# visinf/fldr-vfi

Measured on AMD Instinct MI355X. Metric: 4K frame-pairs interpolated/sec, higher is better.
Workload: dtype f32 (3x3 convs: 3 x fp16-split MFMA with fp32 accumulation — error against fp64 within 1.5x (mean) / 2x (max) of the exact fp32-MFMA kernel's on every layer shape, tests/test_gpu_parity.py::test_split_fp16_conv_is_fp32_equivalent; rest fp32/fp64)

## Files before the change

### fldr-vfi_amd/csrc/splat_acc64_kernels.hip

```cpp
#include "splat_common.h"

#define SA_SBQ 64
#define SA_Q 512
#ifndef SA_WHOLE_PIXELS
#define SA_WHOLE_PIXELS 2304
#endif
#ifndef SA_IMG_TW
#define SA_IMG_TW 64
#define SA_IMG_TH 24
#define SA_IMG_K 3
#define SA_IMG_U 4
#endif
#ifndef SA_IMGQ_U
#define SA_IMGQ_U 1
#endif
#ifndef SA_FEAT_TW
#define SA_FEAT_TW 32
#define SA_FEAT_TH 8
#define SA_FEAT_K 1
#define SA_FEAT_U 1
#endif

typedef _Float16 sa_h8 __attribute__((ext_vector_type(8)));

struct SaProblem {
    const float* img;
    const float* flow;
    const float* metric;
    const float* blk;
    const float* sbt;
    float* out_f32;
    unsigned char* out_spk;
    int64_t img_bstride, img_cstride, flow_bstride;
};
struct SaArgs {
    SaProblem p[2];
    int N, C, H, W, groups, nsb_x, nsb;
    int whole;
    int gpw;
    int tiles_x, st_y, n_st, total, per_xcd;
};

template <int CB, int U, bool QUAD>
struct SaBuf {
    int x[U], y[U];
    bool ok[U];
    float fx[U], fy[U], mv[U], val[U][CB];
};
template <int CB, int U>
struct SaBuf<CB, U, true> {
    int x[U], y[U];
    bool ok[U];
    float4 fx[U], fy[U], mv[U], val[U][CB];
};
__device__ __forceinline__ void sa_pin4(float4& v) { fldr_pin(v.x); fldr_pin(v.y); fldr_pin(v.z); fldr_pin(v.w); }
__device__ __forceinline__ float sa_at(const float4& v, int j) { return j == 0 ? v.x : (j == 1 ? v.y : (j == 2 ? v.z : v.w)); }

template <int MODE, int CB, int TW, int TH, int K, int U, bool QUAD>
__global__ __launch_bounds__(256) void splat_acc64_kernel(SaArgs a) {
#pragma clang fp contract(off)
    constexpr int CA = MODE >= 1 ? CB + 1 : CB;
    constexpr int CELLS = TW * TH;
    extern __shared__ __attribute__((aligned(16))) unsigned char sa_smem[];
    double* acc = reinterpret_cast<double*>(sa_smem);
    int* blkq = reinterpret_cast<int*>(sa_smem + (size_t)CA * CELLS * 8);
    float* redf = reinterpret_cast<float*>(blkq + SA_Q);
    int* redi = reinterpret_cast<int*>(redf + 16);
    int* cnt = redi + 16;
    unsigned short* sbq = reinterpret_cast<unsigned short*>(cnt + 2);

    const int tid = threadIdx.x, lane = tid & 63;
    const int wv = __builtin_amdgcn_readfirstlane(tid >> 6);
    const int lin = (int)(blockIdx.x & 7) * a.per_xcd + (int)(blockIdx.x >> 3);
    if ((int)(blockIdx.x >> 3) >= a.per_xcd || lin >= a.total) return;
    const int zi = lin / a.n_st, st = lin - zi * a.n_st;
    const int sty = st / a.tiles_x, stx = st - sty * a.tiles_x;
    const int wg_groups = a.groups / a.gpw;
    const int per_prob = a.N * wg_groups;
    const int prob = zi / per_prob;
    const int rem = zi - prob * per_prob;
    const int n = rem / wg_groups, grp0 = (rem - n * wg_groups) * a.gpw;
    const SaProblem& P = a.p[prob];
    const int C = a.C, H = a.H, W = a.W, nsb_x = a.nsb_x, nsb = a.nsb;
    int cbase = grp0 * CB;
    const int tx0 = stx * TW, sy0 = sty * (K * TH);
    const int64_t HW = (int64_t)H * W;
    const float ftx0 = (float)tx0, ftx1 = (float)(tx0 + TW - 1), fsy0 = (float)sy0, fsy1 = (float)(min(sy0 + K * TH, H) - 1);
    const float INF = __builtin_inff();

    const float* sbn = P.sbt + (int64_t)n * nsb * 4;
    const float* bkn = P.blk + (int64_t)n * nsb * ST_SB_BLOCKS * 4;
    const bool small = nsb <= SA_SBQ;
    if (tid < 2) cnt[tid] = small && tid == 0 ? nsb : 0;
    if (small && tid < nsb) sbq[tid] = (unsigned short)tid;
    float4 b_first = make_float4(0.0f, 0.0f, 0.0f, 0.0f);
    if (!small && !a.whole) b_first = *reinterpret_cast<const float4*>(sbn + (tid < nsb ? tid : 0) * 4);
    for (int i = tid; i < CA * CELLS / 2; i += 256) reinterpret_cast<double2*>(acc)[i] = make_double2(0.0, 0.0);
    if ((CA * CELLS) & 1) { if (tid == 0) acc[CA * CELLS - 1] = 0.0; }
    __syncthreads();
    if (!small && !a.whole) {
        for (int s = tid; s < nsb; s += 256) {
            const float4 b = s == tid ? b_first : *reinterpret_cast<const float4*>(sbn + s * 4);
            const int sx = (s % nsb_x) * (ST_SBX * ST_BW), sy = (s / nsb_x) * (ST_SBY * ST_BH);
            if (st_match(b, (float)sx, (float)(sx + ST_SBX * ST_BW - 1), (float)sy, (float)(sy + ST_SBY * ST_BH - 1), ftx0, ftx1, fsy0, fsy1)) {
                const int i = atomicAdd(&cnt[0], 1);
                if (i < SA_SBQ) sbq[i] = (unsigned short)s;
            }
        }
        __syncthreads();
    }
    const int n_sb = cnt[0];
    const bool sb_over = a.whole || n_sb > SA_SBQ;
    float rxmin = INF, rxmax = -INF, rymin = INF, rymax = -INF;
    int cx0 = 0x7fffffff, cx1 = -1, cy0 = 0x7fffffff, cy1 = -1;
    if (!sb_over) {
        for (int i = wv; i < n_sb; i += 4) {
            const int s = sbq[i];
            const float4 b = *reinterpret_cast<const float4*>(bkn + ((int64_t)s * ST_SB_BLOCKS + lane) * 4);
            const int bx = (s % nsb_x) * ST_SBX + (lane % ST_SBX), by = (s / nsb_x) * ST_SBY + (lane / ST_SBX);
            const int sx = bx * ST_BW, sy = by * ST_BH;
            if (st_match(b, (float)sx, (float)(sx + ST_BW - 1), (float)sy, (float)(sy + ST_BH - 1), ftx0, ftx1, fsy0, fsy1)) {
                rxmin = fminf(rxmin, b.x); rxmax = fmaxf(rxmax, b.y); rymin = fminf(rymin, b.z); rymax = fmaxf(rymax, b.w);
                cx0 = min(cx0, sx); cx1 = max(cx1, sx + ST_BW - 1); cy0 = min(cy0, sy); cy1 = max(cy1, sy + ST_BH - 1);
                const int k = atomicAdd(&cnt[1], 1);
                if (k < SA_Q) blkq[k] = (by << 16) | bx;
            }
        }
#pragma unroll
        for (int o = 32; o > 0; o >>= 1) {
            rxmin = fminf(rxmin, __shfl_xor(rxmin, o)); rxmax = fmaxf(rxmax, __shfl_xor(rxmax, o));
            rymin = fminf(rymin, __shfl_xor(rymin, o)); rymax = fmaxf(rymax, __shfl_xor(rymax, o));
            cx0 = min(cx0, __shfl_xor(cx0, o)); cx1 = max(cx1, __shfl_xor(cx1, o));
            cy0 = min(cy0, __shfl_xor(cy0, o)); cy1 = max(cy1, __shfl_xor(cy1, o));
        }
        if (lane == 0) {
            redf[wv * 4 + 0] = rxmin; redf[wv * 4 + 1] = rxmax; redf[wv * 4 + 2] = rymin; redf[wv * 4 + 3] = rymax;
            redi[wv * 4 + 0] = cx0; redi[wv * 4 + 1] = cx1; redi[wv * 4 + 2] = cy0; redi[wv * 4 + 3] = cy1;
        }
    }
    __syncthreads();
    int n_match = 0;
    bool bounded = false;
    if (!sb_over) {
        n_match = cnt[1];
#pragma unroll
        for (int k = 0; k < 4; ++k) {
            rxmin = fminf(rxmin, redf[k * 4 + 0]); rxmax = fmaxf(rxmax, redf[k * 4 + 1]);
            rymin = fminf(rymin, redf[k * 4 + 2]); rymax = fmaxf(rymax, redf[k * 4 + 3]);
            cx0 = min(cx0, redi[k * 4 + 0]); cx1 = max(cx1, redi[k * 4 + 1]); cy0 = min(cy0, redi[k * 4 + 2]); cy1 = max(cy1, redi[k * 4 + 3]);
        }
        bounded = fabsf(rxmin) < 1.0e6f && fabsf(rxmax) < 1.0e6f && fabsf(rymin) < 1.0e6f && fabsf(rymax) < 1.0e6f;
    }

    const float* fl = P.flow + (int64_t)n * P.flow_bstride;
    const float* mt = P.metric ? P.metric + (int64_t)n * HW : nullptr;
    const float* inn = P.img + (int64_t)n * P.img_bstride;
    float* on = P.out_f32 ? P.out_f32 + (int64_t)n * C * HW : nullptr;
    const int G = (C + 7) >> 3;
    unsigned char* sp = P.out_spk ? P.out_spk + (int64_t)n * G * 2 * HW * 16 : nullptr;
    bool bad = false;

    int ty0 = 0;
    int X0 = 0, Y0 = 0, Rw = 1, Rh = 0, n_chunks = 0;
    bool rect = true;
    int rx = 0, ry = 0, dqx = 0, dqy = 0;
    auto plan_tile = [&](int k) __attribute__((always_inline)) {
        ty0 = sy0 + k * TH;
        const float fty0 = (float)ty0, fty1 = (float)(ty0 + TH - 1);
        int X1 = W - 1, Y1 = H - 1;
        X0 = 0; Y0 = 0; rect = true; n_chunks = 0;
        if (sb_over) {
            n_chunks = (int)((HW + 255) / 256);
        } else if (n_match > 0) {
            X0 = cx0; X1 = min(cx1, W - 1); Y0 = cy0; Y1 = min(cy1, H - 1);
            if (bounded) {
                X0 = max(X0, (int)floorf(ftx0 - 2.0f - rxmax)); X1 = min(X1, (int)ceilf(ftx1 + 1.0f - rxmin));
                Y0 = max(Y0, (int)floorf(fty0 - 2.0f - rymax)); Y1 = min(Y1, (int)ceilf(fty1 + 1.0f - rymin));
            }
            const int64_t area = (int64_t)max(X1 - X0 + 1, 0) * max(Y1 - Y0 + 1, 0);
            rect = n_match > SA_Q || area <= (int64_t)256 * n_match;
            n_chunks = rect ? (int)((area + 255) / 256) : n_match;
        }
        Rw = max(X1 - X0 + 1, 1); Rh = max(Y1 - Y0 + 1, 0);
        if constexpr (QUAD) {
            X0 &= ~3; X1 = min(X1 | 3, W - 1);
            Rw = max((X1 - X0 + 1) >> 2, 1);
            if (n_chunks > 0) n_chunks = rect ? (int)(((int64_t)Rw * Rh + 255) / 256) : (n_match + 3) >> 2;
        }
        rx = tid % Rw; ry = tid / Rw;
        dqx = 256 % Rw; dqy = 256 / Rw;
#if defined(SA_ABLATE) && SA_ABLATE == 1
        n_chunks = 0;
#endif
    };

    auto load_chunk = [&](SaBuf<CB, U, QUAD>& b, int u, int k) __attribute__((always_inline)) {
        int x, y;
        bool ok;
        if (rect) {
            x = X0 + (QUAD ? 4 * rx : rx); y = Y0 + ry;
            ok = k < n_chunks && ry < Rh;
            rx += dqx; ry += dqy;
            if (rx >= Rw) { rx -= Rw; ++ry; }
        } else if constexpr (QUAD) {
            const int bi = 4 * k + wv;
            const int e = blkq[bi < n_match ? bi : 0];
            x = (e & 0xFFFF) * ST_BW + (lane & 15) * 4; y = (e >> 16) * ST_BH + (lane >> 4);
            ok = bi < n_match && x < W && y < H;
        } else {
            const int e = blkq[k < n_chunks ? k : 0];
            x = (e & 0xFFFF) * ST_BW + lane; y = (e >> 16) * ST_BH + wv;
            ok = k < n_chunks && x < W && y < H;
        }
        b.x[u] = x; b.y[u] = y; b.ok[u] = ok;
        const int64_t pix = ok ? (int64_t)y * W + x : 0;
        if constexpr (QUAD) {
            b.fx[u] = *reinterpret_cast<const float4*>(fl + pix); b.fy[u] = *reinterpret_cast<const float4*>(fl + HW + pix);
            b.mv[u] = make_float4(0.0f, 0.0f, 0.0f, 0.0f);
            if ((MODE == 2 || MODE == 3) && mt != nullptr) b.mv[u] = *reinterpret_cast<const float4*>(mt + pix);
#pragma unroll
            for (int c = 0; c < CB; ++c) {
                const int cc = cbase + c < C ? cbase + c : C - 1;
                b.val[u][c] = *reinterpret_cast<const float4*>(inn + (int64_t)cc * P.img_cstride + pix);
            }
        } else {
            b.fx[u] = fl[pix]; b.fy[u] = fl[HW + pix];
            b.mv[u] = 0.0f;
            if ((MODE == 2 || MODE == 3) && mt != nullptr) b.mv[u] = mt[pix];
#pragma unroll
            for (int c = 0; c < CB; ++c) {
                const int cc = cbase + c < C ? cbase + c : C - 1;
                b.val[u][c] = inn[(int64_t)cc * P.img_cstride + pix];
            }
        }
    };
    auto load_iter = [&](SaBuf<CB, U, QUAD>& b, int k0) __attribute__((always_inline)) {
#pragma unroll
        for (int u = 0; u < U; ++u) load_chunk(b, u, k0 + u);
    };
    auto process = [&](SaBuf<CB, U, QUAD>& b) __attribute__((always_inline)) {
      if constexpr (QUAD) {
#pragma unroll
        for (int u = 0; u < U; ++u) {
            sa_pin4(b.fx[u]); sa_pin4(b.fy[u]); sa_pin4(b.mv[u]);
#pragma unroll
            for (int c = 0; c < CB; ++c) sa_pin4(b.val[u][c]);
        }
#if defined(SA_ABLATE) && SA_ABLATE == 3
        return;
#endif
#pragma unroll
        for (int u = 0; u < U; ++u) {
            if (!b.ok[u]) continue;
            int x0[4], y0[4], iw[4], ie[4];
            float wnw[4], wne[4], wsw[4], wse[4], wg[4];
            bool xa[4], xb[4], ya[4], yb[4];
            bool any = false;
#pragma unroll
            for (int j = 0; j < 4; ++j) {
                const StGeom g = st_geom(b.x[u] + j, b.y[u], sa_at(b.fx[u], j), sa_at(b.fy[u], j), W, H);
                x0[j] = g.x0; y0[j] = g.y0; wnw[j] = g.wnw; wne[j] = g.wne; wsw[j] = g.wsw; wse[j] = g.wse;
                const uint32_t ulx = (uint32_t)(g.x0 - tx0), uly = (uint32_t)(g.y0 - ty0), ux1 = ulx + 1u;
                xa[j] = ulx < (uint32_t)TW; xb[j] = ux1 < (uint32_t)TW; ya[j] = uly < (uint32_t)TH; yb[j] = uly + 1u < (uint32_t)TH;
                iw[j] = (int)(uly * (uint32_t)TW + (ulx & 3u) * (uint32_t)(TW / 4) + (ulx >> 2));
                ie[j] = (int)(uly * (uint32_t)TW + (ux1 & 3u) * (uint32_t)(TW / 4) + (ux1 >> 2));
                any = any || ((xa[j] || xb[j]) && (ya[j] || yb[j]));
                wg[j] = 1.0f;
                if (MODE == 2) wg[j] = sa_at(b.mv[u], j);
                if (MODE == 3 && mt != nullptr) wg[j] = expf(sa_at(b.mv[u], j));
            }
            if (!any) continue;
            float v[4][CA];
#pragma unroll
            for (int j = 0; j < 4; ++j)
#pragma unroll
                for (int c = 0; c < CA; ++c) {
                    float t = wg[j];
                    if (c < CB) {
                        t = sa_at(b.val[u][c < CB ? c : 0], j);
                        if (MODE == 3) t = (t + 1.0f) / 2.0f;
                        if (MODE >= 2) t = t * wg[j];
                        if (cbase + c >= C) t = 0.0f;
                    }
                    v[j][c] = t;
                }
            bool gn[4], gs[4];
#pragma unroll
            for (int j = 0; j < 4; ++j) {
                const bool coh = j < 3 && x0[j] + 1 == x0[j < 3 ? j + 1 : j] && y0[j] == y0[j < 3 ? j + 1 : j];
                gn[j] = coh && xb[j] && ya[j]; gs[j] = coh && xb[j] && yb[j];
            }
#pragma unroll
            for (int j = 0; j < 4; ++j) {
                const int jp = j > 0 ? j - 1 : 0;
                if (xa[j] && ya[j]) {
#pragma unroll
                    for (int c = 0; c < CA; ++c) {
                        double d = (double)(v[j][c] * wnw[j]);
                        if (j > 0) d += (double)(gn[jp] ? v[jp][c] * wne[jp] : 0.0f);
                        atomicAdd(acc + c * CELLS + iw[j], d);
                    }
                }
                if (xa[j] && yb[j]) {
#pragma unroll
                    for (int c = 0; c < CA; ++c) {
                        double d = (double)(v[j][c] * wsw[j]);
                        if (j > 0) d += (double)(gs[jp] ? v[jp][c] * wse[jp] : 0.0f);
                        atomicAdd(acc + c * CELLS + iw[j] + TW, d);
                    }
                }
                if (xb[j] && ya[j] && !gn[j]) {
#pragma unroll
                    for (int c = 0; c < CA; ++c) atomicAdd(acc + c * CELLS + ie[j], (double)(v[j][c] * wne[j]));
                }
                if (xb[j] && yb[j] && !gs[j]) {
#pragma unroll
                    for (int c = 0; c < CA; ++c) atomicAdd(acc + c * CELLS + ie[j] + TW, (double)(v[j][c] * wse[j]));
                }
            }
        }
      } else {
#pragma unroll
        for (int u = 0; u < U; ++u) {
            fldr_pin(b.fx[u]); fldr_pin(b.fy[u]); fldr_pin(b.mv[u]);
#pragma unroll
            for (int c = 0; c < CB; ++c) fldr_pin(b.val[u][c]);
        }
#if defined(SA_ABLATE) && SA_ABLATE == 3
        return;
#endif
#pragma unroll
        for (int u = 0; u < U; ++u) {
            if (!b.ok[u]) continue;
            const StGeom g = st_geom(b.x[u], b.y[u], b.fx[u], b.fy[u], W, H);
            const int lx = g.x0 - tx0, ly = g.y0 - ty0;
            if (lx < -1 || lx >= TW || ly < -1 || ly >= TH) continue;
            const bool cxa = lx >= 0 && g.x0 < W, cxb = lx + 1 < TW && g.x0 + 1 < W;
            const bool cya = ly >= 0 && g.y0 < H, cyb = ly + 1 < TH && g.y0 + 1 < H;
            const bool vnw = cxa && cya, vne = cxb && cya, vsw = cxa && cyb, vse = cxb && cyb;
            float wgt = 1.0f;
            if (MODE == 2) wgt = b.mv[u];
            if (MODE == 3 && mt != nullptr) wgt = expf(b.mv[u]);
            double* cell = acc + (ly * TW + lx);
#pragma unroll
            for (int c = 0; c < CA; ++c) {
                float v;
                if (c < CB) {
                    v = b.val[u][c];
                    if (MODE == 3) v = (v + 1.0f) / 2.0f;
                    if (MODE >= 2) v = v * wgt;
                    if (cbase + c >= C) v = 0.0f;
                } else {
                    v = wgt;
                }
                double* pc = cell + c * CELLS;
#if defined(SA_ABLATE) && SA_ABLATE == 2
                asm volatile("" :: "v"(pc), "v"(v * g.wnw), "v"(v * g.wne), "v"(v * g.wsw), "v"(v * g.wse), "v"((int)vnw + (int)vne + (int)vsw + (int)vse));
#else
                if (vnw) atomicAdd(pc, (double)(v * g.wnw));
                if (vne) atomicAdd(pc + 1, (double)(v * g.wne));
                if (vsw) atomicAdd(pc + TW, (double)(v * g.wsw));
                if (vse) atomicAdd(pc + TW + 1, (double)(v * g.wse));
#endif
            }
        }
      }
    };
    auto finish = [&](int fy0, int cbase) __attribute__((always_inline)) {
      if constexpr (QUAD) {
        static_assert(!QUAD || (CB % 8 != 0 && TW % 4 == 0), "the run walk serves the image configuration (fp32 output)");
        for (int i = tid; i < CELLS / 4; i += 256) {
            const int xq = i % (TW / 4), yy = i / (TW / 4);
            const int x = tx0 + 4 * xq, y = fy0 + yy;
            const int cell = yy * TW + xq;
            float norm[4] = {1.0f, 1.0f, 1.0f, 1.0f};
            if (MODE >= 1) {
#pragma unroll
                for (int j = 0; j < 4; ++j) {
                    norm[j] = (float)acc[CB * CELLS + cell + j * (TW / 4)]; acc[CB * CELLS + cell + j * (TW / 4)] = 0.0;
                    if (norm[j] == 0.0f) norm[j] = 1.0f;
                }
            }
            float o[CB][4];
            StRecip rn[4];
            bool fast = true;
            if (MODE >= 1) {
#pragma unroll
                for (int j = 0; j < 4; ++j) { rn[j] = st_recip(norm[j]); fast = fast && st_recip_safe(norm[j]); }
                fast = __builtin_amdgcn_ballot_w64(!fast) == 0ull;
            }
#pragma unroll
            for (int c = 0; c < CB; ++c)
#pragma unroll
                for (int j = 0; j < 4; ++j) {
                    float v = (float)acc[c * CELLS + cell + j * (TW / 4)];
                    acc[c * CELLS + cell + j * (TW / 4)] = 0.0;
                    if (MODE >= 1) v = fast ? st_div(v, rn[j]) : v / norm[j];
                    o[c][j] = (v - 0.5f) * 2.0f;
                }
            if (x >= W || y >= H || !on) continue;
            const int64_t pix = (int64_t)y * W + x;
#pragma unroll
            for (int c = 0; c < CB; ++c)
                if (cbase + c < C) *reinterpret_cast<float4*>(on + (int64_t)(cbase + c) * HW + pix) = make_float4(o[c][0], o[c][1], o[c][2], o[c][3]);
        }
      } else {
        for (int i = tid; i < CELLS; i += 256) {
            const int x = tx0 + i % TW, y = fy0 + i / TW;
            float norm = 1.0f;
            if (MODE >= 1) { norm = (float)acc[CB * CELLS + i]; acc[CB * CELLS + i] = 0.0; if (norm == 0.0f) norm = 1.0f; }
            float o[CB];
            const StRecip rn = st_recip(norm);
            const bool fast = MODE >= 1 && __builtin_amdgcn_ballot_w64(!st_recip_safe(norm)) == 0ull;
#pragma unroll
            for (int c = 0; c < CB; ++c) {
                float v = (float)acc[c * CELLS + i];
                acc[c * CELLS + i] = 0.0;
                if (MODE >= 1) v = fast ? st_div(v, rn) : v / norm;
                o[c] = cbase + c < C ? (v - 0.5f) * 2.0f : 0.0f;
            }
            if (x >= W || y >= H) continue;
            const int64_t pix = (int64_t)y * W + x;
            if (on) {
#pragma unroll
                for (int c = 0; c < CB; ++c)
                    if (cbase + c < C) on[(int64_t)(cbase + c) * HW + pix] = o[c];
            }
            if constexpr (CB % 8 == 0) {
                if (sp) {
#pragma unroll
                    for (int g8 = 0; g8 < CB / 8; ++g8) {
                        const int gi = (cbase >> 3) + g8;
                        if (gi >= G) break;
                        sa_h8 hi, lo;
                        {
                            float xs[8];
                            _Float16 hs[8], ls[8];
#pragma unroll
                            for (int k = 0; k < 8; ++k) xs[k] = o[g8 * 8 + k];
                            fldr_split_hl_group(xs, hs, ls, bad);
#pragma unroll
                            for (int k = 0; k < 8; ++k) { hi[k] = hs[k]; lo[k] = ls[k]; }
                        }
                        unsigned char* d = sp + ((int64_t)gi * 2 * HW + pix) * 16;
                        *reinterpret_cast<sa_h8*>(d) = hi;
                        *reinterpret_cast<sa_h8*>(d + HW * 16) = lo;
                    }
                }
            }
        }
      }
    };

    SaBuf<CB, U, QUAD> b0, b1;
    const int n_units = K * a.gpw;
    auto begin_unit = [&](int u) __attribute__((always_inline)) {
        const int k = u / a.gpw;
        cbase = (grp0 + (u - k * a.gpw)) * CB;
        plan_tile(k);
        if (n_chunks > 0) load_iter(b0, 0);
    };
    begin_unit(0);
#pragma unroll 1
    for (int u = 0; u < n_units; ++u) {
        const int cur_y0 = ty0, cur_cbase = cbase;
        if (cur_y0 >= H) break;
        for (int k0 = 0; k0 < n_chunks; k0 += 2 * U) {
            const bool more = k0 + U < n_chunks;
            if (more) load_iter(b1, k0 + U);
            process(b0);
            if (!more) break;
            if (k0 + 2 * U < n_chunks) load_iter(b0, k0 + 2 * U);
            process(b1);
        }
        const bool next = u + 1 < n_units && sy0 + ((u + 1) / a.gpw) * TH < H;
        if (next) begin_unit(u + 1);
        __syncthreads();
        finish(cur_y0, cur_cbase);
        if (!next) break;
        __syncthreads();
    }
    fldr_note_range(bad);
}

FLDR_TU_STATUS(acc64)

#ifndef SA_FOLD_MIN_TILES
#define SA_FOLD_MIN_TILES 512
#endif
#ifndef SA_QUAD_DEFAULT
#define SA_QUAD_DEFAULT 1
#endif
static int g_sa_quad = SA_QUAD_DEFAULT;
FLDR_HOOK int fldr_debug_splat_quad(int v) { if (v == 0 || v == 1) g_sa_quad = v; return g_sa_quad; }
static int g_sa_group_fold = 0;
FLDR_HOOK int fldr_debug_splat_group_fold(int v) { if (v == 0 || v == 1) g_sa_group_fold = v; return g_sa_group_fold; }

template <int MODE, int CB, int TW, int TH, int K, int U, bool QUAD = false>
static int sa_launch2(SaArgs& a, int nprob, hipStream_t s) {
    constexpr int CA = MODE >= 1 ? CB + 1 : CB;
    constexpr int LDS = CA * TW * TH * 8 + SA_Q * 4 + 16 * 4 + 16 * 4 + 2 * 4 + SA_SBQ * 2;
    static_assert(LDS <= 160 * 1024, "tile does not fit the LDS");
    static std::atomic<uint64_t> attr_done{0};
    if (int e = fldr_set_max_lds(reinterpret_cast<const void*>(&splat_acc64_kernel<MODE, CB, TW, TH, K, U, QUAD>), LDS, attr_done)) return e;
    a.tiles_x = fldr_cdiv(a.W, TW);
    a.st_y = fldr_cdiv(a.H, K * TH);
    a.n_st = a.tiles_x * a.st_y;
    const int64_t total = (int64_t)nprob * a.N * (a.groups / a.gpw) * a.n_st;
    if (total > (1ll << 30)) return FLDR_E_SHAPE;
    a.total = (int)total;
    a.per_xcd = (a.total + 7) / 8;
    hipLaunchKernelGGL((splat_acc64_kernel<MODE, CB, TW, TH, K, U, QUAD>), dim3(8 * a.per_xcd), dim3(256), LDS, s, a);
    return 0;
}

template <int MODE>
static int sa_launch(SaArgs& a, int nprob, hipStream_t s) {
    if (a.C <= 3) {
        a.groups = 1; a.gpw = 1;
        bool quad = g_sa_quad && a.W % 4 == 0;
        for (int k = 0; k < nprob && quad; ++k) {
            const SaProblem& p = a.p[k];
            quad = ((reinterpret_cast<uintptr_t>(p.img) | reinterpret_cast<uintptr_t>(p.flow) | reinterpret_cast<uintptr_t>(p.metric) |
                     reinterpret_cast<uintptr_t>(p.out_f32)) & 15) == 0 && ((p.img_bstride | p.img_cstride | p.flow_bstride) & 3) == 0 && p.out_spk == nullptr;
        }
        if (quad) return sa_launch2<MODE, 3, SA_IMG_TW, SA_IMG_TH, SA_IMG_K, SA_IMGQ_U, true>(a, nprob, s);
        return sa_launch2<MODE, 3, SA_IMG_TW, SA_IMG_TH, SA_IMG_K, SA_IMG_U>(a, nprob, s);
    }
    a.groups = fldr_cdiv(a.C, 16);
    const int64_t tiles = (int64_t)nprob * a.N * fldr_cdiv(a.W, SA_FEAT_TW) * fldr_cdiv(a.H, SA_FEAT_TH * SA_FEAT_K);
    a.gpw = (g_sa_group_fold && tiles >= SA_FOLD_MIN_TILES) ? a.groups : 1;
    return sa_launch2<MODE, 16, SA_FEAT_TW, SA_FEAT_TH, SA_FEAT_K, SA_FEAT_U>(a, nprob, s);
}

extern "C" int fldr_softsplat_acc64(const fldr_splat_acc_desc* d, fldr_stream_t stream) {
    FLDR_CHECK_ARG(d && d->nprob >= 1 && d->nprob <= 2 && d->N > 0 && d->C > 0 && d->H > 0 && d->W > 0 && d->mode >= 0 && d->mode <= 3);
    FLDR_CHECK_ARG(!(d->flags & ~7) && (!(d->flags & 2) || (d->nprob == 2 && !(d->flags & 1))));
    if (d->W > 65535 * ST_BW || d->H > 32767 * ST_BH || (int64_t)d->H * d->W * 4 >= (1ll << 32)) return FLDR_E_SHAPE;
    if ((int64_t)fldr_cdiv(d->W, ST_SBX * ST_BW) * fldr_cdiv(d->H, ST_SBY * ST_BH) > 65535) return FLDR_E_SHAPE;
    SaArgs a;
    a.N = d->N; a.C = d->C; a.H = d->H; a.W = d->W; a.groups = 1;
    a.whole = ((d->flags & 4) || (!(d->flags & 3) && (int64_t)d->H * d->W <= SA_WHOLE_PIXELS)) ? 1 : 0;
    a.nsb_x = fldr_cdiv(d->W, ST_SBX * ST_BW);
    a.nsb = a.nsb_x * fldr_cdiv(d->H, ST_SBY * ST_BH);
    hipStream_t s = fldr_s(stream);
    const int64_t HW = (int64_t)d->H * d->W;
    for (int k = 0; k < 2; ++k) {
        const int j = k < d->nprob ? k : 0;
        FLDR_CHECK_ARG(d->img[j] && d->flow[j] && (a.whole || d->ws[(d->flags & 2) ? 0 : j]) && (d->out_f32[j] || d->out_spk[j]));
        FLDR_CHECK_ARG(d->mode != 2 || d->metric[j] != nullptr);
        FLDR_CHECK_ARG(!d->out_spk[j] || d->C > 3);
        SaProblem& p = a.p[k];
        p.img = d->img[j]; p.flow = d->flow[j]; p.metric = d->metric[j];
        if (a.whole) {
            p.blk = p.sbt = nullptr;
// ... 24 lines not shown
```

### fldr-vfi_amd/csrc/splat_common.h

```cpp
#pragma once
#include "common.h"

#define ST_BW 64
#define ST_BH 4
#define ST_SBX 4
#define ST_SBY 16
#define ST_SB_BLOCKS (ST_SBX * ST_SBY)
#define ST_Q 1024
#define ST_SBQ 64
#define ST_U 4

struct StGeom {
    int   x0, y0;
    float wnw, wne, wsw, wse;
};

__device__ __forceinline__ StGeom st_geom(int x, int y, float fx, float fy, int W, int H) {
#pragma clang fp contract(off)
    StGeom g;
    float ox = (float)x + fx;
    float oy = (float)y + fy;
    float xf = floorf(ox), yf = floorf(oy);
    float x1 = xf + 1.0f, y1 = yf + 1.0f;
    g.wnw = (x1 - ox) * (y1 - oy);
    g.wne = (ox - xf) * (y1 - oy);
    g.wsw = (x1 - ox) * (oy - yf);
    g.wse = (ox - xf) * (oy - yf);
    xf = fminf(fmaxf(xf, -2.0f), (float)W + 1.0f);
    yf = fminf(fmaxf(yf, -2.0f), (float)H + 1.0f);
    g.x0 = (int)xf; g.y0 = (int)yf;
    return g;
}

struct StRecip { float n, r; };
__device__ __forceinline__ StRecip st_recip(float n) {
    StRecip q;
    q.n = n;
    const float r0 = __builtin_amdgcn_rcpf(n);
// ... 95 lines not shown
```

### fldr-vfi_amd/fldr_hip.py

```python
import ctypes
import os

import torch

_HERE = os.path.dirname(os.path.abspath(__file__))
LIB_PATH = os.environ.get("FLDR_LIB") or os.path.join(_HERE, "libfldr_hip.so")

MAX_SRC = 12
_c_float_p = ctypes.c_void_p


class ConvDesc(ctypes.Structure):
    _fields_ = [
        ("src", ctypes.c_void_p * MAX_SRC),
        ("src_bstride", ctypes.c_int64 * MAX_SRC),
        ("src_c", ctypes.c_int32 * MAX_SRC),
        ("src_up2", ctypes.c_int32 * MAX_SRC),
        ("n_src", ctypes.c_int32),
        ("wpack", ctypes.c_void_p),
        ("bias", ctypes.c_void_p),
        ("residual", ctypes.c_void_p),
        ("out", ctypes.c_void_p),
        ("N", ctypes.c_int32), ("cin", ctypes.c_int32), ("cout", ctypes.c_int32), ("cout_store", ctypes.c_int32),
        ("Hin", ctypes.c_int32), ("Win", ctypes.c_int32), ("Hout", ctypes.c_int32), ("Wout", ctypes.c_int32),
# ... 99 lines not shown
    "fldr_debug_s2_vec4": (ctypes.c_int, [ctypes.c_int]),
    "fldr_bwarp": (ctypes.c_int, [_c_float_p] * 3 + [ctypes.c_int] * 5 + [ctypes.c_void_p]),
    "fldr_bwarp_tscaled": (ctypes.c_int, [_c_float_p] * 4 + [ctypes.c_int] * 7 + [ctypes.c_void_p]),
    "fldr_resize_bilinear": (ctypes.c_int, [_c_float_p] * 2 + [ctypes.c_int] * 5 + [ctypes.c_float, ctypes.c_void_p]),
    "fldr_level0_prep": (ctypes.c_int, [ctypes.POINTER(PrepDesc), ctypes.c_void_p]),
    "fldr_zmetric": (ctypes.c_int, [_c_float_p] * 3 + [ctypes.c_float, _c_float_p] + [ctypes.c_int] * 4 + [ctypes.c_void_p]),
    "fldr_conv_prepack_size": (ctypes.c_int64, [ctypes.c_int] * 3),
    "fldr_conv_prepack": (ctypes.c_int, [_c_float_p] * 2 + [ctypes.c_int] * 3 + [ctypes.c_void_p]),
    "fldr_conv2d": (ctypes.c_int, [ctypes.POINTER(ConvDesc), ctypes.c_void_p]),
    "fldr_conv_split_prepack_size": (ctypes.c_int64, [ctypes.c_int] * 2),
    "fldr_conv_split_prepack": (ctypes.c_int, [_c_float_p] * 2 + [ctypes.c_int] * 2 + [ctypes.c_void_p]),
    "fldr_conv2d_split": (ctypes.c_int, [ctypes.POINTER(ConvDesc), ctypes.c_void_p]),
    "fldr_conv_s2_prepack_size": (ctypes.c_int64, [ctypes.c_int] * 2),
    "fldr_conv_s2_prepack": (ctypes.c_int, [_c_float_p] * 2 + [ctypes.c_int] * 2 + [ctypes.c_void_p]),
    "fldr_conv2d_s2_split": (ctypes.c_int, [ctypes.POINTER(ConvDesc), ctypes.c_void_p]),
    "fldr_conv2d_s2_spk": (ctypes.c_int, [ctypes.POINTER(ConvDesc), ctypes.c_void_p]),
    "fldr_conv2d_s2_spk_pair": (ctypes.c_int, [ctypes.POINTER(ConvDesc), ctypes.POINTER(ConvDesc), ctypes.c_void_p]),
    "fldr_debug_s2_persistent": (ctypes.c_int, [ctypes.c_int]),
    "fldr_debug_s2_dma": (ctypes.c_int, [ctypes.c_int]),
    "fldr_debug_s2_xshift": (ctypes.c_int, [ctypes.c_int]),
    "fldr_debug_dec3_xshift": (ctypes.c_int, [ctypes.c_int]),
    "fldr_debug_dec3_xcd": (ctypes.c_int, [ctypes.c_int]),
    "fldr_debug_splat_quad": (ctypes.c_int, [ctypes.c_int]),
    "fldr_spk_bytes": (ctypes.c_int64, [ctypes.c_int] * 3),
    "fldr_spk_pack": (ctypes.c_int, [_c_float_p, ctypes.c_int64, ctypes.c_void_p] + [ctypes.c_int] * 4 + [ctypes.c_void_p]),
    "fldr_spk_unpack": (ctypes.c_int, [ctypes.c_void_p, _c_float_p] + [ctypes.c_int] * 4 + [ctypes.c_void_p]),
    "fldr_conv_spk_prepack_size": (ctypes.c_int64, [ctypes.c_int] * 2),
    "fldr_conv_spk_prepack": (ctypes.c_int, [_c_float_p] * 2 + [ctypes.c_int] * 2 + [ctypes.c_void_p]),
    "fldr_conv2d_spk": (ctypes.c_int, [ctypes.POINTER(SpkConvDesc), ctypes.c_void_p]),
    "fldr_conv2d_spk_levels": (ctypes.c_int, [ctypes.POINTER(SpkConvDesc), ctypes.c_int, ctypes.c_void_p]),
    "fldr_debug_spk_wgs_per_xcd": (ctypes.c_int, [ctypes.c_int]),
    "fldr_range_status": (ctypes.c_int, [ctypes.c_int]),
    "fldr_ring_status": (ctypes.c_int, [ctypes.c_int]),
    "fldr_debug_spk_small_units": (ctypes.c_int, [ctypes.c_int]),
    "fldr_debug_spk_variant": (ctypes.c_int, [ctypes.c_int]),
    "fldr_debug_ring_consumers": (ctypes.c_int, [ctypes.c_int]),
    "fldr_debug_ring32": (ctypes.c_int, [ctypes.c_int]),
    "fldr_debug_ring_resident": (ctypes.c_int, [ctypes.c_int]),
    "fldr_debug_ring_timeouts": (ctypes.c_int, []),
    "fldr_debug_busy_partner": (ctypes.c_int, [ctypes.c_void_p, ctypes.c_int, ctypes.c_int, ctypes.c_int, ctypes.c_int, ctypes.c_void_p]),
    "fldr_sizeof_desc": (ctypes.c_int, [ctypes.c_int]),
    "fldr_synth_tail": (ctypes.c_int, [_c_float_p, ctypes.POINTER(ctypes.c_void_p), ctypes.POINTER(ctypes.c_int64),
                                       _c_float_p, ctypes.c_double, _c_float_p, _c_float_p] + [ctypes.c_int] * 3 + [ctypes.c_void_p]),
    "fldr_dec3_prepack": (ctypes.c_int, [_c_float_p, _c_float_p, ctypes.c_void_p]),
    "fldr_dec3_synth": (ctypes.c_int, [_c_float_p] * 3 + [ctypes.POINTER(ctypes.c_void_p), ctypes.POINTER(ctypes.c_int64),
                                       _c_float_p, ctypes.c_double, _c_float_p, _c_float_p, _c_float_p] + [ctypes.c_int] * 3 + [ctypes.c_void_p]),
# ... 1190 lines not shown
```

### include/fldr_hip_test_hooks.h

```cpp
#ifndef FLDR_HIP_TEST_HOOKS_H
#define FLDR_HIP_TEST_HOOKS_H
#include "fldr_hip.h"
#ifdef __cplusplus
extern "C" {
#endif

FLDR_API int fldr_debug_pca_variant(int v);
FLDR_API int fldr_debug_pca_workgroups(int v);
FLDR_API int fldr_debug_s2_persistent(int v);
FLDR_API int fldr_debug_s2_xshift(int v);
FLDR_API int fldr_debug_s2_vec4(int v);
FLDR_API int fldr_debug_dec3_xshift(int v);
FLDR_API int fldr_debug_splat_quad(int v);
FLDR_API int fldr_debug_dec3_xcd(int v);
FLDR_API int fldr_debug_spk_small_units(int v);
FLDR_API int fldr_debug_spk_wgs_per_xcd(int v);
FLDR_API int fldr_debug_spk_variant(int v);
FLDR_API int fldr_debug_ring_resident(int v);
FLDR_API int fldr_debug_ring32(int v);
FLDR_API int fldr_debug_ring_consumers(int v);
FLDR_API int fldr_debug_corr_variant(int v);
FLDR_API int fldr_debug_corr_xcd(int v);
FLDR_API int fldr_debug_corr_chunk(int v);
FLDR_API int fldr_debug_ring_tile_width(int v);
FLDR_API int fldr_debug_ring_spin_limit(int v);
FLDR_API int64_t fldr_debug_ringrow_pack_floats(int cout, int cin);
FLDR_API int fldr_debug_ringrow_prepack(const float* weight, const float* wpack, float* wrow, int cout, int cin, fldr_stream_t stream);
FLDR_API int fldr_debug_conv2d_ringrow(const fldr_spk_conv_desc* desc, const float* wrow, fldr_stream_t stream);
FLDR_API int fldr_debug_busy_partner(float* out, int workgroups, int lds_bytes, int iters, int kind, fldr_stream_t stream);
FLDR_API int fldr_debug_ring_timeouts(void);
FLDR_API int fldr_debug_splat_tile_variant(int v);
FLDR_API int fldr_debug_pca_variant(int v);
FLDR_API int fldr_debug_pca_workgroups(int v);
FLDR_API int fldr_debug_s2_persistent(int v);
FLDR_API int fldr_debug_s2_xshift(int v);
FLDR_API int fldr_debug_s2_vec4(int v);
// ... 19 lines not shown
```

Before: 523.0.

## Parameterize splat workgroup size, add early corner culling and visit counters

The splat accumulation kernel gets a templated workgroup size, and the block-list chunking packs several blocks per chunk when more waves are available. The quad path now computes the cheap corner positions first and skips the full bilinear geometry and value setup when no corner lands in the tile. It also interleaves weight computation with the atomics to cut register pressure. Test-hook-only counters record visit and hit statistics. The quad path's unit count no longer multiplies by group folding. Defaults keep 256 threads, so the main runtime change is the early cull and per-corner restructuring.

```diff
diff --git a/fldr-vfi_amd/csrc/splat_acc64_kernels.hip b/fldr-vfi_amd/csrc/splat_acc64_kernels.hip
--- a/fldr-vfi_amd/csrc/splat_acc64_kernels.hip
+++ b/fldr-vfi_amd/csrc/splat_acc64_kernels.hip
@@ -11,6 +11,12 @@
 #define SA_IMG_K 3
 #define SA_IMG_U 4
 #endif
+#ifndef SA_IMGQ_TW
+#define SA_IMGQ_TW 64
+#define SA_IMGQ_TH 24
+#define SA_IMGQ_K 3
+#define SA_IMGQ_NT 256
+#endif
 #ifndef SA_IMGQ_U
 #define SA_IMGQ_U 1
 #endif
@@ -19,9 +25,17 @@
 #define SA_FEAT_TH 8
 #define SA_FEAT_K 1
 #define SA_FEAT_U 1
+#define SA_FEAT_NT 256
 #endif
 
 typedef _Float16 sa_h8 __attribute__((ext_vector_type(8)));
+
+#ifdef FLDR_TEST_HOOKS
+#define SA_COUNT(...) __VA_ARGS__
+#else
+#define SA_COUNT(...)
+#endif
+#define SA_NVISIT 8
 
 struct SaProblem {
     const float* img;
@@ -39,6 +53,9 @@
     int whole;
     int gpw;
     int tiles_x, st_y, n_st, total, per_xcd;
+#ifdef FLDR_TEST_HOOKS
+    unsigned long long* visits;
+#endif
 };
 
 template <int CB, int U, bool QUAD>
@@ -56,17 +73,20 @@
 __device__ __forceinline__ void sa_pin4(float4& v) { fldr_pin(v.x); fldr_pin(v.y); fldr_pin(v.z); fldr_pin(v.w); }
 __device__ __forceinline__ float sa_at(const float4& v, int j) { return j == 0 ? v.x : (j == 1 ? v.y : (j == 2 ? v.z : v.w)); }
 
-template <int MODE, int CB, int TW, int TH, int K, int U, bool QUAD>
-__global__ __launch_bounds__(256) void splat_acc64_kernel(SaArgs a) {
+template <int MODE, int CB, int TW, int TH, int K, int U, bool QUAD, int NT>
+__global__ __launch_bounds__(NT) void splat_acc64_kernel(SaArgs a) {
 #pragma clang fp contract(off)
     constexpr int CA = MODE >= 1 ? CB + 1 : CB;
     constexpr int CELLS = TW * TH;
+    constexpr int NW = NT / 64;
+    constexpr int BPC = QUAD ? NW : NW / ST_BH;
+    static_assert(NT % 64 == 0 && BPC >= 1 && (QUAD || NW % ST_BH == 0), "workgroup size");
     extern __shared__ __attribute__((aligned(16))) unsigned char sa_smem[];
     double* acc = reinterpret_cast<double*>(sa_smem);
     int* blkq = reinterpret_cast<int*>(sa_smem + (size_t)CA * CELLS * 8);
     float* redf = reinterpret_cast<float*>(blkq + SA_Q);
-    int* redi = reinterpret_cast<int*>(redf + 16);
-    int* cnt = redi + 16;
+    int* redi = reinterpret_cast<int*>(redf + 4 * NW);
+    int* cnt = redi + 4 * NW;
     unsigned short* sbq = reinterpret_cast<unsigned short*>(cnt + 2);
 
     const int tid = threadIdx.x, lane = tid & 63;
@@ -95,11 +115,11 @@
     if (small && tid < nsb) sbq[tid] = (unsigned short)tid;
     float4 b_first = make_float4(0.0f, 0.0f, 0.0f, 0.0f);
     if (!small && !a.whole) b_first = *reinterpret_cast<const float4*>(sbn + (tid < nsb ? tid : 0) * 4);
-    for (int i = tid; i < CA * CELLS / 2; i += 256) reinterpret_cast<double2*>(acc)[i] = make_double2(0.0, 0.0);
+    for (int i = tid; i < CA * CELLS / 2; i += NT) reinterpret_cast<double2*>(acc)[i] = make_double2(0.0, 0.0);
     if ((CA * CELLS) & 1) { if (tid == 0) acc[CA * CELLS - 1] = 0.0; }
     __syncthreads();
     if (!small && !a.whole) {
-        for (int s = tid; s < nsb; s += 256) {
+        for (int s = tid; s < nsb; s += NT) {
             const float4 b = s == tid ? b_first : *reinterpret_cast<const float4*>(sbn + s * 4);
             const int sx = (s % nsb_x) * (ST_SBX * ST_BW), sy = (s / nsb_x) * (ST_SBY * ST_BH);
             if (st_match(b, (float)sx, (float)(sx + ST_SBX * ST_BW - 1), (float)sy, (float)(sy + ST_SBY * ST_BH - 1), ftx0, ftx1, fsy0, fsy1)) {
@@ -114,7 +134,7 @@
     float rxmin = INF, rxmax = -INF, rymin = INF, rymax = -INF;
     int cx0 = 0x7fffffff, cx1 = -1, cy0 = 0x7fffffff, cy1 = -1;
     if (!sb_over) {
-        for (int i = wv; i < n_sb; i += 4) {
+        for (int i = wv; i < n_sb; i += NW) {
             const int s = sbq[i];
             const float4 b = *reinterpret_cast<const float4*>(bkn + ((int64_t)s * ST_SB_BLOCKS + lane) * 4);
             const int bx = (s % nsb_x) * ST_SBX + (lane % ST_SBX), by = (s / nsb_x) * ST_SBY + (lane / ST_SBX);
@@ -144,7 +164,7 @@
     if (!sb_over) {
         n_match = cnt[1];
 #pragma unroll
-        for (int k = 0; k < 4; ++k) {
+        for (int k = 0; k < NW; ++k) {
             rxmin = fminf(rxmin, redf[k * 4 + 0]); rxmax = fmaxf(rxmax, redf[k * 4 + 1]);
             rymin = fminf(rymin, redf[k * 4 + 2]); rymax = fmaxf(rymax, redf[k * 4 + 3]);
             cx0 = min(cx0, redi[k * 4 + 0]); cx1 = max(cx1, redi[k * 4 + 1]); cy0 = min(cy0, redi[k * 4 + 2]); cy1 = max(cy1, redi[k * 4 + 3]);
@@ -152,6 +172,7 @@
         bounded = fabsf(rxmin) < 1.0e6f && fabsf(rxmax) < 1.0e6f && fabsf(rymin) < 1.0e6f && fabsf(rymax) < 1.0e6f;
     }
 
+    SA_COUNT(unsigned n_vis = 0, n_any = 0, n_dst = 0;)
     const float* fl = P.flow + (int64_t)n * P.flow_bstride;
     const float* mt = P.metric ? P.metric + (int64_t)n * HW : nullptr;
     const float* inn = P.img + (int64_t)n * P.img_bstride;
@@ -170,7 +191,7 @@
         int X1 = W - 1, Y1 = H - 1;
         X0 = 0; Y0 = 0; rect = true; n_chunks = 0;
         if (sb_over) {
-            n_chunks = (int)((HW + 255) / 256);
+            n_chunks = (int)((HW + NT - 1) / NT);
         } else if (n_match > 0) {
             X0 = cx0; X1 = min(cx1, W - 1); Y0 = cy0; Y1 = min(cy1, H - 1);
             if (bounded) {
@@ -178,17 +199,17 @@
                 Y0 = max(Y0, (int)floorf(fty0 - 2.0f - rymax)); Y1 = min(Y1, (int)ceilf(fty1 + 1.0f - rymin));
             }
             const int64_t area = (int64_t)max(X1 - X0 + 1, 0) * max(Y1 - Y0 + 1, 0);
-            rect = n_match > SA_Q || area <= (int64_t)256 * n_match;
-            n_chunks = rect ? (int)((area + 255) / 256) : n_match;
+            rect = n_match > SA_Q || area <= (int64_t)(ST_BW * ST_BH) * n_match;
+            n_chunks = rect ? (int)((area + NT - 1) / NT) : (n_match + BPC - 1) / BPC;
         }
         Rw = max(X1 - X0 + 1, 1); Rh = max(Y1 - Y0 + 1, 0);
         if constexpr (QUAD) {
             X0 &= ~3; X1 = min(X1 | 3, W - 1);
             Rw = max((X1 - X0 + 1) >> 2, 1);
-            if (n_chunks > 0) n_chunks = rect ? (int)(((int64_t)Rw * Rh + 255) / 256) : (n_match + 3) >> 2;
+            if (n_chunks > 0 && rect) n_chunks = (int)(((int64_t)Rw * Rh + NT - 1) / NT);
         }
         rx = tid % Rw; ry = tid / Rw;
-        dqx = 256 % Rw; dqy = 256 / Rw;
+        dqx = NT % Rw; dqy = NT / Rw;
 #if defined(SA_ABLATE) && SA_ABLATE == 1
         n_chunks = 0;
 #endif
@@ -203,14 +224,15 @@
             rx += dqx; ry += dqy;
             if (rx >= Rw) { rx -= Rw; ++ry; }
         } else if constexpr (QUAD) {
-            const int bi = 4 * k + wv;
+            const int bi = NW * k + wv;
             const int e = blkq[bi < n_match ? bi : 0];
             x = (e & 0xFFFF) * ST_BW + (lane & 15) * 4; y = (e >> 16) * ST_BH + (lane >> 4);
             ok = bi < n_match && x < W && y < H;
         } else {
-            const int e = blkq[k < n_chunks ? k : 0];
-            x = (e & 0xFFFF) * ST_BW + lane; y = (e >> 16) * ST_BH + wv;
-            ok = k < n_chunks && x < W && y < H;
+            const int bi = BPC * k + wv / ST_BH;
+            const int e = blkq[bi < n_match ? bi : 0];
+            x = (e & 0xFFFF) * ST_BW + lane; y = (e >> 16) * ST_BH + wv % ST_BH;
+            ok = bi < n_match && x < W && y < H;
         }
         b.x[u] = x; b.y[u] = y; b.ok[u] = ok;
         const int64_t pix = ok ? (int64_t)y * W + x : 0;
@@ -252,71 +274,69 @@
 #pragma unroll
         for (int u = 0; u < U; ++u) {
             if (!b.ok[u]) continue;
-            int x0[4], y0[4], iw[4], ie[4];
-            float wnw[4], wne[4], wsw[4], wse[4], wg[4];
-            bool xa[4], xb[4], ya[4], yb[4];
+            int x0[4], y0[4];
             bool any = false;
+#pragma unroll
+            for (int j = 0; j < 4; ++j) {
+                x0[j] = st_corner(b.x[u] + j, sa_at(b.fx[u], j), W); y0[j] = st_corner(b.y[u], sa_at(b.fy[u], j), H);
+                const uint32_t ulx = (uint32_t)(x0[j] - tx0), uly = (uint32_t)(y0[j] - ty0);
+                any = any || ((ulx < (uint32_t)TW || ulx + 1u < (uint32_t)TW) && (uly < (uint32_t)TH || uly + 1u < (uint32_t)TH));
+            }
+            SA_COUNT(n_vis += 1; n_any += any ? 1 : 0;)
+            if (!any) continue;
+            float hn[CA], hs[CA];
+            bool gn = false, gs = false;
 #pragma unroll
             for (int j = 0; j < 4; ++j) {
                 const StGeom g = st_geom(b.x[u] + j, b.y[u], sa_at(b.fx[u], j), sa_at(b.fy[u], j), W, H);
-                x0[j] = g.x0; y0[j] = g.y0; wnw[j] = g.wnw; wne[j] = g.wne; wsw[j] = g.wsw; wse[j] = g.wse;
-                const uint32_t ulx = (uint32_t)(g.x0 - tx0), uly = (uint32_t)(g.y0 - ty0), ux1 = ulx + 1u;
-                xa[j] = ulx < (uint32_t)TW; xb[j] = ux1 < (uint32_t)TW; ya[j] = uly < (uint32_t)TH; yb[j] = uly + 1u < (uint32_t)TH;
-                iw[j] = (int)(uly * (uint32_t)TW + (ulx & 3u) * (uint32_t)(TW / 4) + (ulx >> 2));
-                ie[j] = (int)(uly * (uint32_t)TW + (ux1 & 3u) * (uint32_t)(TW / 4) + (ux1 >> 2));
-                any = any || ((xa[j] || xb[j]) && (ya[j] || yb[j]));
-                wg[j] = 1.0f;
-                if (MODE == 2) wg[j] = sa_at(b.mv[u], j);
-                if (MODE == 3 && mt != nullptr) wg[j] = expf(sa_at(b.mv[u], j));
-            }
-            if (!any) continue;
-            float v[4][CA];
-#pragma unroll
-            for (int j = 0; j < 4; ++j)
+                const uint32_t ulx = (uint32_t)(x0[j] - tx0), uly = (uint32_t)(y0[j] - ty0), ux1 = ulx + 1u;
+                const bool xa = ulx < (uint32_t)TW, xb = ux1 < (uint32_t)TW, ya = uly < (uint32_t)TH, yb = uly + 1u < (uint32_t)TH;
+                const int iw = (int)(uly * (uint32_t)TW + (ulx & 3u) * (uint32_t)(TW / 4) + (ulx >> 2));
+                const int ie = (int)(uly * (uint32_t)TW + (ux1 & 3u) * (uint32_t)(TW / 4) + (ux1 >> 2));
+                const bool coh = j < 3 && x0[j] + 1 == x0[j < 3 ? j + 1 : j] && y0[j] == y0[j < 3 ? j + 1 : j];
+                const bool gn_j = coh && xb && ya, gs_j = coh && xb && yb;
+                float wg = 1.0f;
+                if (MODE == 2) wg = sa_at(b.mv[u], j);
+                if (MODE == 3 && mt != nullptr) wg = expf(sa_at(b.mv[u], j));
+                float v[CA];
 #pragma unroll
                 for (int c = 0; c < CA; ++c) {
-                    float t = wg[j];
+                    float t = wg;
                     if (c < CB) {
                         t = sa_at(b.val[u][c < CB ? c : 0], j);
                         if (MODE == 3) t = (t + 1.0f) / 2.0f;
-                        if (MODE >= 2) t = t * wg[j];
+                        if (MODE >= 2) t = t * wg;
                         if (cbase + c >= C) t = 0.0f;
                     }
-                    v[j][c] = t;
-                }
-            bool gn[4], gs[4];
-#pragma unroll
-            for (int j = 0; j < 4; ++j) {
-                const bool coh = j < 3 && x0[j] + 1 == x0[j < 3 ? j + 1 : j] && y0[j] == y0[j < 3 ? j + 1 : j];
-                gn[j] = coh && xb[j] && ya[j]; gs[j] = coh && xb[j] && yb[j];
-            }
-#pragma unroll
-            for (int j = 0; j < 4; ++j) {
-                const int jp = j > 0 ? j - 1 : 0;
-                if (xa[j] && ya[j]) {
+                    v[c] = t;
+                }
+                if (xa && ya) {
 #pragma unroll
                     for (int c = 0; c < CA; ++c) {
-                        double d = (double)(v[j][c] * wnw[j]);
-                        if (j > 0) d += (double)(gn[jp] ? v[jp][c] * wne[jp] : 0.0f);
-                        atomicAdd(acc + c * CELLS + iw[j], d);
+                        double d = (double)(v[c] * g.wnw);
+                        if (j > 0) d += (double)(gn ? hn[c] : 0.0f);
+                        atomicAdd(acc + c * CELLS + iw, d);
                     }
                 }
-                if (xa[j] && yb[j]) {
+                if (xa && yb) {
 #pragma unroll
                     for (int c = 0; c < CA; ++c) {
-                        double d = (double)(v[j][c] * wsw[j]);
-                        if (j > 0) d += (double)(gs[jp] ? v[jp][c] * wse[jp] : 0.0f);
-                        atomicAdd(acc + c * CELLS + iw[j] + TW, d);
+                        double d = (double)(v[c] * g.wsw);
+                        if (j > 0) d += (double)(gs ? hs[c] : 0.0f);
+                        atomicAdd(acc + c * CELLS + iw + TW, d);
                     }
                 }
-                if (xb[j] && ya[j] && !gn[j]) {
-#pragma unroll
-                    for (int c = 0; c < CA; ++c) atomicAdd(acc + c * CELLS + ie[j], (double)(v[j][c] * wne[j]));
-                }
-                if (xb[j] && yb[j] && !gs[j]) {
-#pragma unroll
-                    for (int c = 0; c < CA; ++c) atomicAdd(acc + c * CELLS + ie[j] + TW, (double)(v[j][c] * wse[j]));
-                }
+                if (xb && ya && !gn_j) {
+#pragma unroll
+                    for (int c = 0; c < CA; ++c) atomicAdd(acc + c * CELLS + ie, (double)(v[c] * g.wne));
+                }
+                if (xb && yb && !gs_j) {
+#pragma unroll
+                    for (int c = 0; c < CA; ++c) atomicAdd(acc + c * CELLS + ie + TW, (double)(v[c] * g.wse));
+                }
+                gn = gn_j; gs = gs_j;
+#pragma unroll
+                for (int c = 0; c < CA; ++c) { hn[c] = v[c] * g.wne; hs[c] = v[c] * g.wse; }
             }
         }
       } else {
@@ -334,6 +354,7 @@
             if (!b.ok[u]) continue;
             const StGeom g = st_geom(b.x[u], b.y[u], b.fx[u], b.fy[u], W, H);
             const int lx = g.x0 - tx0, ly = g.y0 - ty0;
+            SA_COUNT(n_vis += 1; n_any += (lx < -1 || lx >= TW || ly < -1 || ly >= TH) ? 0 : 1;)
             if (lx < -1 || lx >= TW || ly < -1 || ly >= TH) continue;
             const bool cxa = lx >= 0 && g.x0 < W, cxb = lx + 1 < TW && g.x0 + 1 < W;
             const bool cya = ly >= 0 && g.y0 < H, cyb = ly + 1 < TH && g.y0 + 1 < H;
@@ -369,7 +390,7 @@
     auto finish = [&](int fy0, int cbase) __attribute__((always_inline)) {
       if constexpr (QUAD) {
         static_assert(!QUAD || (CB % 8 != 0 && TW % 4 == 0), "the run walk serves the image configuration (fp32 output)");
-        for (int i = tid; i < CELLS / 4; i += 256) {
+        for (int i = tid; i < CELLS / 4; i += NT) {
             const int xq = i % (TW / 4), yy = i / (TW / 4);
             const int x = tx0 + 4 * xq, y = fy0 + yy;
             const int cell = yy * TW + xq;
@@ -398,6 +419,7 @@
                     if (MODE >= 1) v = fast ? st_div(v, rn[j]) : v / norm[j];
                     o[c][j] = (v - 0.5f) * 2.0f;
                 }
+            SA_COUNT(n_dst += (x < W && y < H) ? 4 : 0;)
             if (x >= W || y >= H || !on) continue;
             const int64_t pix = (int64_t)y * W + x;
 #pragma unroll
@@ -405,7 +427,7 @@
                 if (cbase + c < C) *reinterpret_cast<float4*>(on + (int64_t)(cbase + c) * HW + pix) = make_float4(o[c][0], o[c][1], o[c][2], o[c][3]);
         }
       } else {
-        for (int i = tid; i < CELLS; i += 256) {
+        for (int i = tid; i < CELLS; i += NT) {
             const int x = tx0 + i % TW, y = fy0 + i / TW;
             float norm = 1.0f;
             if (MODE >= 1) { norm = (float)acc[CB * CELLS + i]; acc[CB * CELLS + i] = 0.0; if (norm == 0.0f) norm = 1.0f; }
@@ -419,6 +441,7 @@
                 if (MODE >= 1) v = fast ? st_div(v, rn) : v / norm;
                 o[c] = cbase + c < C ? (v - 0.5f) * 2.0f : 0.0f;
             }
+            SA_COUNT(n_dst += (x < W && y < H) ? 1 : 0;)
             if (x >= W || y >= H) continue;
             const int64_t pix = (int64_t)y * W + x;
             if (on) {
@@ -453,7 +476,7 @@
     };
 
     SaBuf<CB, U, QUAD> b0, b1;
-    const int n_units = K * a.gpw;
+    const int n_units = QUAD ? K : K * a.gpw;
     auto begin_unit = [&](int u) __attribute__((always_inline)) {
         const int k = u / a.gpw;
         cbase = (grp0 + (u - k * a.gpw)) * CB;
@@ -481,6 +504,17 @@
         __syncthreads();
     }
     fldr_note_range(bad);
+#ifdef FLDR_TEST_HOOKS
+    if (a.visits) {
+#pragma unroll
+        for (int o = 32; o > 0; o >>= 1) { n_vis += __shfl_xor(n_vis, o); n_any += __shfl_xor(n_any, o); n_dst += __shfl_xor(n_dst, o); }
+        unsigned long long* v = a.visits + (CB <= 3 ? 0 : SA_NVISIT);
+        if (lane == 0) {
+            atomicAdd(v + 0, (unsigned long long)n_vis); atomicAdd(v + 1, (unsigned long long)n_any);
+            atomicAdd(v + 2, (unsigned long long)n_vis * (QUAD ? 4 : 1)); atomicAdd(v + 3, (unsigned long long)n_dst);
+        }
+    }
+#endif
 }
 
 FLDR_TU_STATUS(acc64)
@@ -495,14 +529,35 @@
 FLDR_HOOK int fldr_debug_splat_quad(int v) { if (v == 0 || v == 1) g_sa_quad = v; return g_sa_quad; }
 static int g_sa_group_fold = 0;
 FLDR_HOOK int fldr_debug_splat_group_fold(int v) { if (v == 0 || v == 1) g_sa_group_fold = v; return g_sa_group_fold; }
-
-template <int MODE, int CB, int TW, int TH, int K, int U, bool QUAD = false>
+#ifdef FLDR_TEST_HOOKS
+static unsigned long long* g_sa_visits_dev = nullptr;
+static unsigned long long g_sa_visits_host[2 * SA_NVISIT];
+static bool g_sa_count = false;
+FLDR_HOOK int fldr_debug_splat_visits(int v, unsigned long long* out) {
+    if (!g_sa_visits_dev) {
+        if (hipMalloc(&g_sa_visits_dev, 2 * SA_NVISIT * sizeof(unsigned long long)) != hipSuccess) { g_sa_visits_dev = nullptr; return FLDR_E_ARG; }
+        if (hipMemset(g_sa_visits_dev, 0, 2 * SA_NVISIT * sizeof(unsigned long long)) != hipSuccess) return FLDR_E_ARG;
+    }
+    if (out) {
+        if (hipDeviceSynchronize() != hipSuccess || hipMemcpy(out, g_sa_visits_dev, 2 * SA_NVISIT * sizeof(unsigned long long), hipMemcpyDeviceToHost) != hipSuccess) return FLDR_E_ARG;
+        for (int i = 0; i < 2 * SA_NVISIT; ++i) out[i] += g_sa_visits_host[i];
+    }
+    if (v == 0 || v == 1) {
+        if (hipDeviceSynchronize() != hipSuccess || hipMemset(g_sa_visits_dev, 0, 2 * SA_NVISIT * sizeof(unsigned long long)) != hipSuccess) return FLDR_E_ARG;
+        for (int i = 0; i < 2 * SA_NVISIT; ++i) g_sa_visits_host[i] = 0;
+        g_sa_count = v == 1;
+    }
+    return g_sa_count ? 1 : 0;
+}
+#endif
+
+template <int MODE, int CB, int TW, int TH, int K, int U, bool QUAD = false, int NT = 256>
 static int sa_launch2(SaArgs& a, int nprob, hipStream_t s) {
     constexpr int CA = MODE >= 1 ? CB + 1 : CB;
-    constexpr int LDS = CA * TW * TH * 8 + SA_Q * 4 + 16 * 4 + 16 * 4 + 2 * 4 + SA_SBQ * 2;
+    constexpr int LDS = CA * TW * TH * 8 + SA_Q * 4 + 2 * (NT / 64) * 4 * 4 + 2 * 4 + SA_SBQ * 2;
     static_assert(LDS <= 160 * 1024, "tile does not fit the LDS");
     static std::atomic<uint64_t> attr_done{0};
-    if (int e = fldr_set_max_lds(reinterpret_cast<const void*>(&splat_acc64_kernel<MODE, CB, TW, TH, K, U, QUAD>), LDS, attr_done)) return e;
+    if (int e = fldr_set_max_lds(reinterpret_cast<const void*>(&splat_acc64_kernel<MODE, CB, TW, TH, K, U, QUAD, NT>), LDS, attr_done)) return e;
     a.tiles_x = fldr_cdiv(a.W, TW);
     a.st_y = fldr_cdiv(a.H, K * TH);
     a.n_st = a.tiles_x * a.st_y;
@@ -510,7 +565,14 @@
     if (total > (1ll << 30)) return FLDR_E_SHAPE;
     a.total = (int)total;
     a.per_xcd = (a.total + 7) / 8;
-    hipLaunchKernelGGL((splat_acc64_kernel<MODE, CB, TW, TH, K, U, QUAD>), dim3(8 * a.per_xcd), dim3(256), LDS, s, a);
+#ifdef FLDR_TEST_HOOKS
+    a.visits = g_sa_count ? g_sa_visits_dev : nullptr;
+    if (g_sa_count) {
+        unsigned long long* h = g_sa_visits_host + (CB <= 3 ? 0 : SA_NVISIT);
+        h[4] += (unsigned long long)nprob * a.N * a.groups * a.H * a.W; h[5] += 1;
+    }
+#endif
+    hipLaunchKernelGGL((splat_acc64_kernel<MODE, CB, TW, TH, K, U, QUAD, NT>), dim3(8 * a.per_xcd), dim3(NT), LDS, s, a);
     return 0;
 }
 
@@ -524,13 +586,13 @@
             quad = ((reinterpret_cast<uintptr_t>(p.img) | reinterpret_cast<uintptr_t>(p.flow) | reinterpret_cast<uintptr_t>(p.metric) |
                      reinterpret_cast<uintptr_t>(p.out_f32)) & 15) == 0 && ((p.img_bstride | p.img_cstride | p.flow_bstride) & 3) == 0 && p.out_spk == nullptr;
         }
-        if (quad) return sa_launch2<MODE, 3, SA_IMG_TW, SA_IMG_TH, SA_IMG_K, SA_IMGQ_U, true>(a, nprob, s);
+        if (quad) return sa_launch2<MODE, 3, SA_IMGQ_TW, SA_IMGQ_TH, SA_IMGQ_K, SA_IMGQ_U, true, SA_IMGQ_NT>(a, nprob, s);
         return sa_launch2<MODE, 3, SA_IMG_TW, SA_IMG_TH, SA_IMG_K, SA_IMG_U>(a, nprob, s);
     }
     a.groups = fldr_cdiv(a.C, 16);
     const int64_t tiles = (int64_t)nprob * a.N * fldr_cdiv(a.W, SA_FEAT_TW) * fldr_cdiv(a.H, SA_FEAT_TH * SA_FEAT_K);
     a.gpw = (g_sa_group_fold && tiles >= SA_FOLD_MIN_TILES) ? a.groups : 1;
-    return sa_launch2<MODE, 16, SA_FEAT_TW, SA_FEAT_TH, SA_FEAT_K, SA_FEAT_U>(a, nprob, s);
+    return sa_launch2<MODE, 16, SA_FEAT_TW, SA_FEAT_TH, SA_FEAT_K, SA_FEAT_U, false, SA_FEAT_NT>(a, nprob, s);
 }
 
 extern "C" int fldr_softsplat_acc64(const fldr_splat_acc_desc* d, fldr_stream_t stream) {
diff --git a/fldr-vfi_amd/csrc/splat_common.h b/fldr-vfi_amd/csrc/splat_common.h
--- a/fldr-vfi_amd/csrc/splat_common.h
+++ b/fldr-vfi_amd/csrc/splat_common.h
@@ -14,6 +14,11 @@
     int   x0, y0;
     float wnw, wne, wsw, wse;
 };
+
+__device__ __forceinline__ int st_corner(int x, float f, int W) {
+#pragma clang fp contract(off)
+    return (int)fminf(fmaxf(floorf((float)x + f), -2.0f), (float)W + 1.0f);
+}
 
 __device__ __forceinline__ StGeom st_geom(int x, int y, float fx, float fy, int W, int H) {
 #pragma clang fp contract(off)
diff --git a/fldr-vfi_amd/fldr_hip.py b/fldr-vfi_amd/fldr_hip.py
--- a/fldr-vfi_amd/fldr_hip.py
+++ b/fldr-vfi_amd/fldr_hip.py
@@ -145,6 +145,7 @@
     "fldr_debug_dec3_xshift": (ctypes.c_int, [ctypes.c_int]),
     "fldr_debug_dec3_xcd": (ctypes.c_int, [ctypes.c_int]),
     "fldr_debug_splat_quad": (ctypes.c_int, [ctypes.c_int]),
+    "fldr_debug_splat_visits": (ctypes.c_int, [ctypes.c_int, ctypes.c_void_p]),
     "fldr_spk_bytes": (ctypes.c_int64, [ctypes.c_int] * 3),
     "fldr_spk_pack": (ctypes.c_int, [_c_float_p, ctypes.c_int64, ctypes.c_void_p] + [ctypes.c_int] * 4 + [ctypes.c_void_p]),
     "fldr_spk_unpack": (ctypes.c_int, [ctypes.c_void_p, _c_float_p] + [ctypes.c_int] * 4 + [ctypes.c_void_p]),
diff --git a/include/fldr_hip_test_hooks.h b/include/fldr_hip_test_hooks.h
--- a/include/fldr_hip_test_hooks.h
+++ b/include/fldr_hip_test_hooks.h
@@ -12,6 +12,7 @@
 FLDR_API int fldr_debug_s2_vec4(int v);
 FLDR_API int fldr_debug_dec3_xshift(int v);
 FLDR_API int fldr_debug_splat_quad(int v);
+FLDR_API int fldr_debug_splat_visits(int v, unsigned long long* out16);
 FLDR_API int fldr_debug_dec3_xcd(int v);
 FLDR_API int fldr_debug_spk_small_units(int v);
 FLDR_API int fldr_debug_spk_wgs_per_xcd(int v);
```

Result: no change. 521.7, median of 6 (-0.3%).
